# facebookresearch/rela

Hardware: AMD Instinct MI355X
Metric: env-steps/s (Ape-X Atari 84x84x4, actor tick + learner grad-step) (higher is better)
Workload: dtype f32 (f32 operands as 3 exact bf16 parts on bf16 MFMA; f32-accurate); 1 GPU; Ape-X DQN 80x80 envs/GPU, actor+learner on one MI355X, replay 2^20, B=512, A=18, n=3; device-resident static frames; parallelism=single

## Files before the change

### rela_amd/csrc/learner.hip

```cpp
#include "learner_common.h"

using namespace rela_amd;

struct rela_apex_learner {
  int device = 0;
  int A = 0, Bmax = 0;
  float gamma_n = 0.f;
  int optimizer = 0;
  float lr = 0.f, opt_eps = 0.f, clip = 0.f;
  int64_t adam_t = 0;
  int64_t off[13] = {0};
  float *P = nullptr, *PT = nullptr, *G = nullptr, *S1 = nullptr, *S2 = nullptr;
  rela_ffnet *online = nullptr, *target = nullptr;
  float *w2p = nullptr, *w3p = nullptr, *wfcp = nullptr;
  void *ws_on = nullptr, *ws_tmp = nullptr;
  int64_t ws_bytes = 0;
  float *q = nullptr;
  float *td = nullptr, *d_ha = nullptr, *d_h = nullptr, *d_a3 = nullptr, *d_a2 = nullptr, *d_a1 = nullptr;
  float *col = nullptr;
  float *part = nullptr;
  float *cpart = nullptr;
  float *s32 = nullptr;
  double* npart = nullptr;
  float* norm = nullptr;
  float* loss = nullptr;
  bool loaded = false;
  int pend_B = 0, last_B = 0;
  int pend_rows = 0;
  const uint8_t* pend_obs = nullptr;
  hipStream_t side = nullptr;
  hipEvent_t ev[8] = {nullptr};
  float *part_side = nullptr, *cpart_side = nullptr;
  void *frag2 = nullptr, *frag3 = nullptr;
};

namespace {
rela_ffnet_params params_at(const rela_apex_learner* l, float* base) {
  rela_ffnet_params p;
  const float** f = reinterpret_cast<const float**>(&p);
  for (int i = 0; i < 12; ++i) f[i] = base + l->off[i];
  return p;
}

int repack(rela_apex_learner* l, bool online, bool target, hipStream_t s) {
  if (online) {
    const rela_ffnet_params p = params_at(l, l->P);
    FFNetExtraPacks extra;
    extra.w2p = l->w2p, extra.w3p = l->w3p, extra.wfcp = l->wfcp;
    int rc = ffnet_load_extra(l->online, &p, s, extra);
    if (rc != RELA_OK) return rc;
    if (l->frag2) dgfast::pack_frags(l->w2p, l->w3p, l->frag2, l->frag3, s);
  }
  if (target) {
    const rela_ffnet_params p = params_at(l, l->PT);
    int rc = rela_ffnet_load(l->target, &p, 1, s);
    if (rc != RELA_OK) return rc;
  }
  return RELA_OK;
}
}

extern "C" int rela_apex_learner_create(rela_apex_learner** out, int num_action, int max_batch, int multi_step,
                                        float gamma, int optimizer, float lr, float eps, float grad_clip,
                                        int device) {
  RELA_CHECK(out && num_action >= 1 && num_action <= 31 && max_batch >= 1 && multi_step >= 1 &&
                 (optimizer == 0 || optimizer == 1),
             RELA_EINVAL, "rela_apex_learner_create: bad arguments (A=%d batch=%d n=%d optimizer=%d)", num_action,
             max_batch, multi_step, optimizer);
  int ndev = 0;
  if (hipGetDeviceCount(&ndev) != hipSuccess || device < 0 || device >= ndev) {
    set_last_error("rela_apex_learner_create: HIP device %d not available (%d visible); there is no CPU path",
                   device, ndev);
    return RELA_ENODEV;
  }
  DeviceGuard g(device);
  auto* l = new rela_apex_learner();
  l->device = device;
  l->A = num_action;
  l->Bmax = max_batch;
  l->gamma_n = (float)pow((double)gamma, (double)multi_step);
  l->optimizer = optimizer;
  l->lr = lr;
  l->opt_eps = eps;
  l->clip = grad_clip;
  const int64_t cnt[12] = {32 * 256, 32, 64 * 512, 64, 64 * 576, 64, (int64_t)512 * 3136, 512, 512, 1,
                           (int64_t)num_action * 512, num_action};
  for (int i = 0; i < 12; ++i) l->off[i + 1] = l->off[i] + (cnt[i] + 3) / 4 * 4;
  const size_t nb = sizeof(float) * (size_t)l->off[12];
  const size_t B = (size_t)max_batch, A = (size_t)num_action;
  RELA_HIP(hipMalloc(&l->P, nb));
  RELA_HIP(hipMalloc(&l->PT, nb));
  RELA_HIP(hipMalloc(&l->G, nb));
  RELA_HIP(hipMalloc(&l->S1, nb));
  RELA_HIP(hipMalloc(&l->S2, nb));
  RELA_HIP(hipMemset(l->P, 0, nb));
  RELA_HIP(hipMemset(l->PT, 0, nb));
  RELA_HIP(hipMemset(l->G, 0, nb));
  RELA_HIP(hipMemset(l->S1, 0, nb));
  RELA_HIP(hipMemset(l->S2, 0, nb));
  int rc = rela_ffnet_create(&l->online, num_action, device);
  if (rc != RELA_OK) return rc;
  rc = rela_ffnet_create(&l->target, num_action, device);
  if (rc != RELA_OK) return rc;
  ffnet_label_as_learner(l->online);
  ffnet_label_as_learner(l->target);
  ffnet_set_max_rows(l->online, max_batch);
  ffnet_set_max_rows(l->target, max_batch);
  RELA_HIP(hipMalloc(&l->w2p, sizeof(float) * 64 * 512));
  RELA_HIP(hipMalloc(&l->w3p, sizeof(float) * 64 * 576));
  RELA_HIP(hipMalloc(&l->wfcp, sizeof(float) * 512 * 3136));
  l->ws_bytes = std::max(rela_ffnet_workspace_bytes(nullptr, max_batch), rela_ffnet_workspace_bytes(nullptr, 2 * max_batch));
  RELA_HIP(hipMalloc(&l->ws_on, (size_t)l->ws_bytes));
  RELA_HIP(hipMalloc(&l->ws_tmp, (size_t)l->ws_bytes));
  RELA_HIP(hipMalloc(&l->q, sizeof(float) * 3 * B * A));
  RELA_HIP(hipMalloc(&l->td, sizeof(float) * B));
  RELA_HIP(hipMalloc(&l->d_ha, sizeof(float) * B * 32));
  RELA_HIP(hipMalloc(&l->d_h, sizeof(float) * B * 512));
  RELA_HIP(hipMalloc(&l->d_a3, sizeof(float) * B * kA3));
  RELA_HIP(hipMalloc(&l->d_a2, sizeof(float) * B * kA2));
  RELA_HIP(hipMalloc(&l->d_a1, sizeof(float) * B * kA1));
  RELA_HIP(hipMalloc(&l->col, sizeof(float) * trunk_col_floats(B)));
  RELA_HIP(hipMalloc(&l->part, sizeof(float) * kTrunkPartFloats));
  RELA_HIP(hipMalloc(&l->cpart, sizeof(float) * kColsumBlocks * (32 + 512 + 64 + 64 + 32)));
  RELA_HIP(hipMalloc(&l->s32, sizeof(float) * 32));
  RELA_HIP(hipMalloc(&l->npart, sizeof(double) * kNormBlocks));
  RELA_HIP(hipMalloc(&l->norm, sizeof(float) * 2));
  RELA_HIP(hipMalloc(&l->loss, sizeof(float)));
  static const bool lanes = !(getenv("RELA_LEARNER_LANES") && atoi(getenv("RELA_LEARNER_LANES")) == 1);
  if (lanes) {
    RELA_HIP(hipStreamCreateWithFlags(&l->side, hipStreamNonBlocking));
    for (hipEvent_t& e : l->ev) RELA_HIP(hipEventCreateWithFlags(&e, hipEventDisableTiming));
    RELA_HIP(hipMalloc(&l->part_side, sizeof(float) * kTrunkPartFloats));
    RELA_HIP(hipMalloc(&l->cpart_side, sizeof(float) * kColsumBlocks * (32 + 512 + 64 + 64 + 32)));
    RELA_HIP(hipMalloc(&l->frag2, dgfast::kFrag2Bytes));
    RELA_HIP(hipMalloc(&l->frag3, dgfast::kFrag3Bytes));
  }
  *out = l;
  return RELA_OK;
}

extern "C" void rela_apex_learner_destroy(rela_apex_learner* l) {
  if (!l) return;
  DeviceGuard g(l->device);
  (void)hipDeviceSynchronize();
  void* ps[] = {l->P,  l->PT,   l->G,    l->S1,   l->S2,   l->w2p, l->w3p,  l->wfcp,  l->ws_on, l->ws_tmp, l->q,
                l->td, l->d_ha, l->d_h,  l->d_a3, l->d_a2, l->d_a1, l->col, l->part,  l->cpart, l->s32,    l->npart,
                l->norm, l->loss, l->part_side, l->cpart_side, l->frag2, l->frag3};
  for (void* p : ps) (void)hipFree(p);
  for (hipEvent_t e : l->ev)
    if (e) (void)hipEventDestroy(e);
  if (l->side) (void)hipStreamDestroy(l->side);
  rela_ffnet_destroy(l->online);
  rela_ffnet_destroy(l->target);
  delete l;
// ... 196 lines not shown
    ProbHeadWgrad p{};
    p.M = 32, p.N = 512, p.K = Bn;
    p.d_ha = l->d_ha, p.h = w.h, p.g_a_w = Gm[10], p.g_v_w = Gm[8], p.A = A;
    if (g3) (void)gemm3::launch_gemm<Tile3W32>(p, 1, sw, "learner_wgrad_heads");
    else if (g6) (void)gemm3::launch_gemm<Tile6W32>(p, 1, sw, "learner_wgrad_heads");
    else launch_gemm<TileW32>(p, 1, sw, "learner_wgrad_heads");
  }
  sums.add(l->d_ha, Bn, 32, l->s32);
  if (lanes) lane_dep(l->ev[3], s, sw);
  {
    ProbFcDgrad p{};
    p.M = Bn, p.N = 3136, p.K = 512;
    p.d_h = l->d_h, p.wfcp = l->wfcp, p.a3 = w.a3, p.d_a3 = l->d_a3;
    if (g3) (void)gemm3::launch_gemm<Tile3Dgrad>(p, 1, s, "learner_dgrad_fc");
    else if (g6) (void)gemm3::launch_gemm<Tile6Dgrad>(p, 1, s, "learner_dgrad_fc");
    else launch_gemm<TileDgrad>(p, 1, s, "learner_dgrad_fc");
  }
  {
    ProbFcWgrad p{};
    p.M = 512, p.N = 3136, p.K = Bn;
    p.d_h = l->d_h, p.a3 = w.a3, p.g_fc_w = Gm[6];
    if (g3) (void)gemm3::launch_gemm<Tile3Wfc>(p, 1, sw, "learner_wgrad_fc");
    else if (g6) (void)gemm3::launch_gemm<Tile6Wfc>(p, 1, sw, "learner_wgrad_fc");
    else launch_gemm<TileWfc>(p, 1, sw, "learner_wgrad_fc");
  }
  sums.add(l->d_h, Bn, 512, Gm[7]);
  {
    TrunkBwd t{};
    t.Bn = Bn, t.obs = obs, t.a1 = w.a1, t.a2 = w.a2, t.d_a3 = l->d_a3, t.d_a2 = l->d_a2, t.d_a1 = l->d_a1;
    t.col = l->col, t.part = l->part, t.cpart = l->cpart, t.w2p = l->w2p, t.w3p = l->w3p;
    t.g_c1w = Gm[0], t.g_c1b = Gm[1], t.g_c2w = Gm[2], t.g_c2b = Gm[3], t.g_c3w = Gm[4], t.g_c3b = Gm[5];
    t.fast = rela_ffnet_precision(l->online) == 1;
    t.emu = g6;
    if (lanes) {
      t.side = sw, t.ev_da3 = l->ev[4], t.ev_da2 = l->ev[5], t.ev_side = l->ev[6];
      t.part_side = l->part_side, t.cpart_side = l->cpart_side;
      if (t.fast) t.frag2 = l->frag2, t.frag3 = l->frag3;
      t.s32 = l->s32, t.A = A, t.g_a_b = Gm[11], t.g_v_b = Gm[9];
    }
    trunk_backward(t, s, &sums);
    if (!lanes) hipLaunchKernelGGL(head_bias_grad, dim3(1), dim3(32), 0, s, (const float*)l->s32, A, Gm[11], Gm[9]);
  }
  RELA_LAUNCH_CHECK();
  return RELA_OK;
}

extern "C" int rela_apex_learner_apply(rela_apex_learner* l, void* stream_) {
  RELA_CHECK(l && l->loaded, RELA_ESTATE, "rela_apex_learner_apply: parameters were never loaded");
  hipStream_t s = (hipStream_t)stream_;
  DeviceGuard g(l->device);
  OptimState o;
  o.optimizer = l->optimizer, o.lr = l->lr, o.eps = l->opt_eps, o.clip = l->clip, o.adam_t = l->adam_t;
  optimizer_apply(o, l->P, l->G, l->S1, l->S2, l->off[12], l->npart, l->norm, s);
  l->adam_t = o.adam_t;
  RELA_LAUNCH_CHECK();
  return repack(l, true, false, s);
}
```

### rela_amd/csrc/learner_common.h

```cpp
#pragma once
#include <cmath>
#include <cstring>
#include <vector>

#include "common.h"
#include "ffnet_layout.h"
#include "gemm_lds.h"
#include "gemm_bf16x3.h"
#include "prof.h"
#include "dgrad_conv_bf16.h"
#include "wgrad_conv1_bf16.h"
#include "wgrad_conv2_bf16.h"
#include "wgrad_conv3_bf16.h"

namespace rela_amd {
namespace {

using namespace gemm;

using TileDgrad = TileCfg<128, 64, 4, 2, false>;
using TileWfc = TileCfg<128, 64, 4, 2, true>;
using TileW64 = TileCfg<64, 64, 2, 4, true>;
using TileW32 = TileCfg<32, 64, 2, 4, true>;
using Tile3Dgrad = gemm3::TileCfg<128, 64, 4, 2, false>;
using Tile3Wfc = gemm3::TileCfg<128, 64, 4, 2, true>;
using Tile3W64 = gemm3::TileCfg<64, 64, 2, 4, true>;
using Tile3W32 = gemm3::TileCfg<32, 64, 2, 4, true>;
inline bool gemm_bf16x3_on() { return true; }
using Tile6Dgrad = gemm3::TileCfg<128, 64, 4, 2, false, 3>;
using Tile6Wfc = gemm3::TileCfg<128, 64, 4, 2, true, 3>;
using Tile6W64 = gemm3::TileCfg<64, 64, 2, 4, true, 3>;
using Tile6W32 = gemm3::TileCfg<32, 64, 2, 4, true, 3>;


struct ProbHeadDgrad : ProbBase {
  const float *d_ha, *a_w, *v_w, *h;
  float* d_h;
  int A;
  __device__ float4 loadA(int m, int k) const { return m < M ? ld4(d_ha + (size_t)m * 32 + k) : zero4(); }
  __device__ float4 loadB(int k, int n) const {
    if (k < A) return ld4(a_w + (size_t)k * 512 + n);
    if (k == 31) return ld4(v_w + n);
    return zero4();
// ... 426 lines not shown
  reinterpret_cast<float4*>(sq)[i] = sv;
  reinterpret_cast<float4*>(p)[i] = pv;
}
__global__ void adam_update(float* __restrict__ p, const float* __restrict__ g, float* __restrict__ m1,
                            float* __restrict__ m2, int64_t n4, float lr, float b1, float b2, float eps, float bc1,
                            float bc2_sqrt, const float* __restrict__ coef) {
  const int64_t i = (int64_t)blockIdx.x * blockDim.x + threadIdx.x;
  const float cf = coef[1];
  if (i >= n4 || cf < 0.f) return;
  const float4 gv = reinterpret_cast<const float4*>(g)[i];
  float4 av = reinterpret_cast<float4*>(m1)[i], bv = reinterpret_cast<float4*>(m2)[i], pv = reinterpret_cast<float4*>(p)[i];
  auto upd = [&](float gi, float& a, float& b, float& pi) {
    gi = gi * cf;
    a = b1 * a + (1.0f - b1) * gi;
    b = b2 * b + (1.0f - b2) * gi * gi;
    pi -= (lr / bc1) * (a / (sqrtf(b) / bc2_sqrt + eps));
  };
  upd(gv.x, av.x, bv.x, pv.x), upd(gv.y, av.y, bv.y, pv.y), upd(gv.z, av.z, bv.z, pv.z), upd(gv.w, av.w, bv.w, pv.w);
  reinterpret_cast<float4*>(m1)[i] = av;
  reinterpret_cast<float4*>(m2)[i] = bv;
  reinterpret_cast<float4*>(p)[i] = pv;
}


constexpr int kSplitW3 = 28, kSplitW2 = 27, kSplitW1 = 64;
constexpr size_t kTrunkPartFloats = (size_t)w3fast::kMaxBlocks * 64 * 576;
static_assert(kTrunkPartFloats * 4 >= dgfast::kFrag3Bytes && kTrunkPartFloats * 4 >= dgfast::kFrag2Bytes, "frag scratch");
static_assert(kTrunkPartFloats >= (size_t)kSplitW3 * 8 * 64 * 576, "part size (split multiplier up to 8)");
static_assert(kTrunkPartFloats >= (size_t)kSplitW3 * 64 * 576 && kTrunkPartFloats >= (size_t)w1fast::kMaxBlocks * 32 * 256 &&
                  kTrunkPartFloats >= (size_t)w2fast::kMaxBlocks * 64 * 512,
              "part size");
static_assert(kSplitW3 * 64 * 576 >= kSplitW2 * 64 * 512 && kSplitW3 * 64 * 576 >= kSplitW1 * 32 * 256, "part size");
inline size_t trunk_col_floats(size_t frames) { return frames * (size_t)(81 * 512 > 49 * 576 ? 81 * 512 : 49 * 576); }

constexpr int kFastWgradMinFrames = 2048;
struct TrunkBwd {
  int Bn;
  const uint8_t* obs;
  const float *a1, *a2;
  const float* d_a3;
  float *d_a2, *d_a1;
  float* col;
  float* part;
  float* cpart;
  const float *w2p, *w3p;
  float *g_c1w, *g_c1b, *g_c2w, *g_c2b, *g_c3w, *g_c3b;
  bool fast = false;
  bool emu = false;
  hipStream_t side = nullptr;
  hipEvent_t ev_da3 = nullptr, ev_da2 = nullptr, ev_side = nullptr;
  float *part_side = nullptr, *cpart_side = nullptr;
  const void *frag2 = nullptr, *frag3 = nullptr;
  const float* s32 = nullptr;
  float *g_a_b = nullptr, *g_v_b = nullptr;
  int A = 0;
};
inline void lane_dep(hipEvent_t ev, hipStream_t from, hipStream_t to) {
  (void)hipEventRecord(ev, from);
  (void)hipStreamWaitEvent(to, ev, 0);
}

inline void colsum_multi_launch(ColsumJobs& jobs, float* cpart, hipStream_t s) {
  if (jobs.n == 0) return;
  int maxC = 0;
  size_t off = 0;
  for (int j = 0; j < jobs.n; ++j) {
    jobs.part[j] = cpart + off;
    off += (size_t)kColsumBlocks * jobs.C[j];
    maxC = jobs.C[j] > maxC ? jobs.C[j] : maxC;
  }
  ProfScope prof("learner_colsum", s);
  hipLaunchKernelGGL(colsum_partial_multi, dim3(kColsumBlocks, jobs.n), dim3(kLT), 0, s, jobs);
  hipLaunchKernelGGL(colsum_final_multi, dim3(maxC / 4, jobs.n), dim3(kColsumBlocks), 0, s, jobs);
}

inline void colsum_launch(const float* src, int64_t rows, int C, float* cpart, float* out, hipStream_t s) {
  ProfScope prof("learner_colsum", s);
  hipLaunchKernelGGL(colsum_partial, dim3(kColsumBlocks), dim3(kLT), 0, s, src, rows, C, cpart);
  hipLaunchKernelGGL(colsum_final, dim3(C / 4), dim3(kColsumBlocks), 0, s, (const float*)cpart, C, out);
}

inline void trunk_backward(const TrunkBwd& t, hipStream_t s, ColsumJobs* pending = nullptr) {
  const int Bn = t.Bn;
  ColsumJobs own;
  ColsumJobs& jobs = pending ? *pending : own;
  const bool lanes = t.side != nullptr;
  hipStream_t sw = lanes ? t.side : s;
  float* partw = lanes ? t.part_side : t.part;
  if (lanes) lane_dep(t.ev_da3, s, sw);
  const bool fast23 = t.fast && Bn >= kFastWgradMinFrames;
  if (fast23) {
    int blocks = 0;
    {
      ProfScope prof("learner_wgrad_conv3", sw);
      (void)w3fast::launch(t.a2, t.d_a3, Bn, partw, sw, &blocks);
    }
    hipLaunchKernelGGL(reduce_splits, dim3(ceil_div(64 * 576, 256)), dim3(256), 0, sw, (const float*)partw, blocks, 64,
                       576, kRedConv3, t.g_c3w);
  } else {
    ProbW3 p{};
    p.M = 64, p.N = 576, p.K = Bn * 49;
    p.d_out = t.d_a3, p.in = t.a2, p.part = partw;
    static const int mul = 3  ;
    const int split3 = Bn <= 1024 ? kSplitW3 * mul : kSplitW3;
    if (t.fast && gemm_bf16x3_on()) (void)gemm3::launch_gemm<Tile3W64>(p, split3, sw, "learner_wgrad_conv3");
    else if (t.emu) (void)gemm3::launch_gemm<Tile6W64>(p, split3, sw, "learner_wgrad_conv3");
    else launch_gemm<TileW64>(p, split3, sw, "learner_wgrad_conv3");
    hipLaunchKernelGGL(reduce_splits, dim3(ceil_div(64 * 576, 256)), dim3(256), 0, sw, (const float*)partw, split3, 64,
                       576, kRedConv3, t.g_c3w);
  }
  jobs.add(t.d_a3, (int64_t)Bn * 49, 64, t.g_c3b);
  if (t.fast) {
    ProfScope prof("learner_dgrad_conv3", s);
    (void)dgfast::launch_conv3(t.d_a3, t.w3p, t.a2, t.d_a2, Bn, t.part, s, t.frag3);
  } else {
    ProbConvDgrad p{};
    p.M = Bn * 49, p.N = 576, p.K = 64;
    p.d_out = t.d_a3, p.wp = t.w3p, p.col = t.col;
    launch_gemm<TileDgrad>(p, 1, s, "learner_dgrad_conv3");
    ProfScope prof("learner_col2im", s);
    hipLaunchKernelGGL(col2im3, dim3(ceil_div((int64_t)Bn * 81 * 16, 256)), dim3(256), 0, s, (const float*)t.col, t.a2,
                       t.d_a2, Bn);
  }
  if (lanes) lane_dep(t.ev_da2, s, sw);
  if (fast23) {
    int blocks = 0;
    {
      ProfScope prof("learner_wgrad_conv2", sw);
      (void)w2fast::launch(t.a1, t.d_a2, Bn, partw, sw, &blocks);
    }
    hipLaunchKernelGGL(reduce_splits, dim3(ceil_div(64 * 512, 256)), dim3(256), 0, sw, (const float*)partw, blocks, 64,
                       512, kRedConv2, t.g_c2w);
  } else {
    ProbW2 p{};
    p.M = 64, p.N = 512, p.K = Bn * 81;
    p.d_out = t.d_a2, p.in = t.a1, p.part = partw;
    static const int mul = 3  ;
    const int split2 = Bn <= 1024 ? kSplitW2 * mul : kSplitW2;
    if (t.fast && gemm_bf16x3_on()) (void)gemm3::launch_gemm<Tile3W64>(p, split2, sw, "learner_wgrad_conv2");
    else if (t.emu) (void)gemm3::launch_gemm<Tile6W64>(p, split2, sw, "learner_wgrad_conv2");
    else launch_gemm<TileW64>(p, split2, sw, "learner_wgrad_conv2");
    hipLaunchKernelGGL(reduce_splits, dim3(ceil_div(64 * 512, 256)), dim3(256), 0, sw, (const float*)partw, split2, 64,
                       512, kRedConv2, t.g_c2w);
  }
  jobs.add(t.d_a2, (int64_t)Bn * 81, 64, t.g_c2b);
  if (lanes) {
    colsum_multi_launch(jobs, t.cpart_side, sw);
    if (t.s32) hipLaunchKernelGGL(head_bias_grad, dim3(1), dim3(32), 0, sw, t.s32, t.A, t.g_a_b, t.g_v_b);
    jobs.n = 0;
  }
  if (t.fast) {
    ProfScope prof("learner_dgrad_conv2", s);
    (void)dgfast::launch_conv2(t.d_a2, t.w2p, t.a1, t.d_a1, Bn, t.part, s, t.frag2);
  } else {
    ProbConvDgrad p{};
    p.M = Bn * 81, p.N = 512, p.K = 64;
    p.d_out = t.d_a2, p.wp = t.w2p, p.col = t.col;
    launch_gemm<TileDgrad>(p, 1, s, "learner_dgrad_conv2");
    ProfScope prof("learner_col2im", s);
    hipLaunchKernelGGL(col2im2, dim3(ceil_div((int64_t)Bn * 400 * 8, 256)), dim3(256), 0, s, (const float*)t.col, t.a1,
                       t.d_a1, Bn);
  }
  if (t.fast) {
    int blocks = 0;
    {
      ProfScope prof("learner_wgrad_conv1", s);
      (void)w1fast::launch(t.obs, t.d_a1, Bn, t.part, s, &blocks, lanes ? 128 : w1fast::kMaxBlocks);
    }
    hipLaunchKernelGGL(reduce_splits, dim3(ceil_div(32 * 256, 256)), dim3(256), 0, s, (const float*)t.part, blocks, 32,
                       256, kRedConv1, t.g_c1w);
  } else {
    ProbW1 p{};
    p.M = 32, p.N = 256, p.K = Bn * 400;
    p.d_out = t.d_a1, p.obs = t.obs, p.part = t.part;
    if (t.emu) (void)gemm3::launch_gemm<Tile6W32>(p, kSplitW1, s, "learner_wgrad_conv1");
    else launch_gemm<TileW32>(p, kSplitW1, s, "learner_wgrad_conv1");
    hipLaunchKernelGGL(reduce_splits, dim3(ceil_div(32 * 256, 256)), dim3(256), 0, s, (const float*)t.part, kSplitW1, 32,
                       256, kRedConv1, t.g_c1w);
  }
  jobs.add(t.d_a1, (int64_t)Bn * 400, 32, t.g_c1b);
  colsum_multi_launch(jobs, t.cpart, s);
  if (lanes) lane_dep(t.ev_side, sw, s);
}

struct OptimState {
  int optimizer = 0;
  float lr = 0.f, eps = 0.f, clip = 0.f;
  int64_t adam_t = 0;
};
inline void optimizer_apply(OptimState& o, float* P, const float* G, float* S1, float* S2, int64_t n, double* npart,
                            float* norm, hipStream_t s, const unsigned* abort_word = nullptr) {
  ProfScope prof("learner_optimizer", s);
// ... 18 lines not shown
```

### rela_amd/csrc/learner_r2d2.hip

```cpp
#include "gemm_bf16s.h"
#include "learner_common.h"

using namespace rela_amd;

namespace rela_amd {
namespace {

constexpr int kHid = 512, kGates = 2048, kFeat = 3136;
constexpr int kRecSplitF = 4;
constexpr int kRecSplitB = 8;

using TileRows = TileCfg<128, 64, 4, 2, false>;
using TileRec = TileCfg<64, 64, 2, 4, false>;
using TileWg = TileCfg<128, 64, 4, 2, true>;
using TileW32r = TileCfg<32, 64, 2, 4, true>;

struct ProbGateX : ProbBase {
  const float *a3, *wihT, *bias;
  float* gx;
  __device__ float4 loadA(int m, int k) const { return m < M ? ld4(a3 + (size_t)m * kFeat + k) : zero4(); }
  __device__ float4 loadB(int k, int n) const { return ld4(wihT + (size_t)k * kGates + n); }
  __device__ void store(int, int m, int n, float v) const { gx[(size_t)m * kGates + n] = v + bias[n]; }
};
struct ProbRecFwd : ProbBase {
// ... 473 lines not shown
  const int idx = blockIdx.x * blockDim.x + threadIdx.x;
  if (idx >= rows * 32) return;
  const int r = idx >> 5, k = idx & 31;
  const float g = dqa[r];
  float v = 0.f;
  if (k < A) v = legal[(size_t)r * A + k] * (g * ((k == (int)act[r] ? 1.0f : 0.0f) - 1.0f / (float)A));
  if (k == 31) v = g;
  d_ha[idx] = v;
}

}
}

struct rela_r2d2_learner {
  int device = 0;
  int A = 0, Bmax = 0, seq = 0, burn = 0, n = 0, T = 0;
  float gamma_n = 0.f, eta = 0.f, one_minus_eta = 0.f;
  OptimState opt;
  int64_t off[15] = {0};
  float *P = nullptr, *PT = nullptr, *G = nullptr, *S1 = nullptr, *S2 = nullptr;
  rela_lstmnet *online = nullptr, *target = nullptr;
  float *w2p = nullptr, *w3p = nullptr;
  float *wihT[2] = {nullptr, nullptr}, *whhT[2] = {nullptr, nullptr}, *bsum[2] = {nullptr, nullptr};
  float* wihp = nullptr;
  float *a1 = nullptr, *a2 = nullptr, *a3 = nullptr;
  float* gxs[2] = {nullptr, nullptr};
  float*& gx = gxs[0];
  float *Hs[2] = {nullptr, nullptr}, *Cs[2] = {nullptr, nullptr};
  float* rec_part = nullptr;
  unsigned* rec_bar = nullptr;
  unsigned* rec_chain_bar = nullptr;
  bool rec_chains_fit = true;
  bool rec_persist = true;
  int precision = 0;
  uint8_t* wrec[2] = {nullptr, nullptr};
  uint8_t* wTrec = nullptr;
  uint8_t *arec = nullptr, *trec = nullptr;
  uint64_t wver[2] = {1, 1}, rec_ver[2] = {0, 0};
  uint8_t* s3rec = nullptr;
  void* wx3[2] = {nullptr, nullptr};
  uint64_t x3_ver[2] = {0, 0};
  float *ha = nullptr, *q_on = nullptr, *q_tg = nullptr;
  float *qmin = nullptr, *qa_on = nullptr, *qa_tg = nullptr, *dqa = nullptr, *d_ha = nullptr, *d_o = nullptr;
  float *dc_rec = nullptr;
  float *d_a3 = nullptr, *d_a2 = nullptr, *d_a1 = nullptr, *col = nullptr, *part = nullptr, *cpart = nullptr,
        *s32 = nullptr;
  double* npart = nullptr;
  float *norm = nullptr, *loss = nullptr, *loss_seq = nullptr;
  bool loaded = false;
  int pend_B = 0;
  const uint8_t* pend_obs = nullptr;
};

namespace {
const int64_t* seg_counts(int A, int64_t cnt[14]) {
  const int64_t c[14] = {32 * 256, 32, 64 * 512, 64, 64 * 576, 64, (int64_t)kGates * kFeat, (int64_t)kGates * kHid,
                         kGates, kGates, 512, 1, (int64_t)A * 512, A};
  for (int i = 0; i < 14; ++i) cnt[i] = c[i];
  return cnt;
}

rela_lstmnet_params lparams_at(const rela_r2d2_learner* l, float* base) {
  rela_lstmnet_params p;
  const float** f = reinterpret_cast<const float**>(&p);
  for (int i = 0; i < 14; ++i) f[i] = base + l->off[i];
  return p;
// ... 148 lines not shown
    }
    ca.term = term, ca.tmo = l->rec_bar, ca.bar = l->rec_chain_bar, ca.T = T, ca.Tpad = Tpad, ca.Bn = Bn, ca.burn = burn;
    ProfScope prof("learner_lstm_rec_persist", s);
    hipLaunchKernelGGL(lstm_rec_chain<true>, dim3(8 * kChainBlocks), dim3(kRecThreads), 0, s, ca);
    RELA_LAUNCH_CHECK();
  } else {
    rc = forward_rec_steps(l, 1, Bn, term, false, s);
    if (rc != RELA_OK) return rc;
    rc = forward_rec_steps(l, 0, Bn, term, true, s);
    if (rc != RELA_OK) return rc;
  }
  const size_t blk = (size_t)Bn * kHid;
  rc = lstmnet_heads(l->target, Tt * Bn, l->Hs[1] + (size_t)(burn + 1) * blk, legal_train, l->ha, l->q_tg, s,
                     "learner_fwd_heads");
  if (rc != RELA_OK) return rc;
  return lstmnet_heads(l->online, Tt * Bn, l->Hs[0] + (size_t)(burn + 1) * blk, legal_train, l->ha, l->q_on, s,
                       "learner_fwd_heads");
}
}

extern "C" int rela_r2d2_learner_create(rela_r2d2_learner** out, int num_action, int max_batch, int multi_step,
                                        float gamma, int seq_len, int burn_in, double eta, int optimizer, float lr,
                                        float eps, float grad_clip, int device) {
  RELA_CHECK(out && num_action >= 1 && num_action <= 31 && max_batch >= 1 && max_batch <= 1024 && multi_step >= 1 &&
                 seq_len >= 1 && burn_in >= 0 && (optimizer == 0 || optimizer == 1),
             RELA_EINVAL, "rela_r2d2_learner_create: bad arguments (A=%d batch=%d n=%d seq=%d burn=%d optimizer=%d)",
             num_action, max_batch, multi_step, seq_len, burn_in, optimizer);
  int ndev = 0;
  if (hipGetDeviceCount(&ndev) != hipSuccess || device < 0 || device >= ndev) {
    set_last_error("rela_r2d2_learner_create: HIP device %d not available (%d visible); there is no CPU path", device,
                   ndev);
    return RELA_ENODEV;
  }
  DeviceGuard g(device);
  auto* l = new rela_r2d2_learner();
  l->device = device;
  l->A = num_action, l->Bmax = max_batch, l->seq = seq_len, l->burn = burn_in, l->n = multi_step;
  l->T = burn_in + seq_len + multi_step;
  l->gamma_n = (float)pow((double)gamma, (double)multi_step);
  l->eta = (float)eta;
  l->one_minus_eta = (float)(1.0 - eta);
  l->opt.optimizer = optimizer, l->opt.lr = lr, l->opt.eps = eps, l->opt.clip = grad_clip;
  int64_t cnt[14];
  seg_counts(num_action, cnt);
  for (int i = 0; i < 14; ++i) l->off[i + 1] = l->off[i] + (cnt[i] + 3) / 4 * 4;
  const size_t nb = sizeof(float) * (size_t)l->off[14];
  const size_t B = (size_t)max_batch, A = (size_t)num_action, T = (size_t)l->T, Tt = T - burn_in;
  const size_t rowsAll = T * B, rowsTr = Tt * B;
  auto alloc = [&](float** p, size_t floats, bool zero) -> int {
    RELA_HIP(hipMalloc(p, sizeof(float) * floats));
    if (zero) RELA_HIP(hipMemset(*p, 0, sizeof(float) * floats));
    return RELA_OK;
  };
#define R2_ALLOC(ptr, floats, zero)               \
  do {                                            \
    int _rc = alloc(&(ptr), (floats), (zero));    \
    if (_rc != RELA_OK) return _rc;               \
  } while (0)
  R2_ALLOC(l->P, l->off[14], true);
  R2_ALLOC(l->PT, l->off[14], true);
  R2_ALLOC(l->G, l->off[14], true);
  R2_ALLOC(l->S1, l->off[14], true);
  R2_ALLOC(l->S2, l->off[14], true);
  (void)nb;
  int rc = rela_lstmnet_create(&l->online, num_action, device);
  if (rc != RELA_OK) return rc;
  rc = rela_lstmnet_create(&l->target, num_action, device);
  if (rc != RELA_OK) return rc;
  R2_ALLOC(l->w2p, 64 * 512, false);
// ... 38 lines not shown
    const size_t f = (size_t)kRecSplitF * B * kGates, b = (size_t)kRecSplitB * B * kHid;
    R2_ALLOC(l->rec_part, f > b ? f : b, false);
  }
  RELA_HIP(hipMalloc(&l->rec_bar, sizeof(unsigned) * (size_t)(8 + 2 * ((T + 3) / 4 * 4))));
  RELA_HIP(hipMemset(l->rec_bar, 0, sizeof(unsigned) * (size_t)(8 + 2 * ((T + 3) / 4 * 4))));
  RELA_HIP(hipMalloc(&l->rec_chain_bar, sizeof(unsigned) * (size_t)(8 * ((T + 3) / 4 * 4))));
  l->rec_persist = !(getenv("RELA_R2D2_REC") && strcmp(getenv("RELA_R2D2_REC"), "steps") == 0);
  if (l->rec_persist) {
    int cus = 0;
    RELA_HIP(hipDeviceGetAttribute(&cus, hipDeviceAttributeMultiprocessorCount, device));
    int occ_c = 0, occ_d = 0;
    if (hipOccupancyMaxActiveBlocksPerMultiprocessor(&occ_c, lstm_rec_chain<true>, kRecThreads, 0) != hipSuccess) occ_c = 0;
    if (hipOccupancyMaxActiveBlocksPerMultiprocessor(&occ_d, lstm_bptt_chain<false>, kRecThreads, 0) != hipSuccess) occ_d = 0;
    auto room = [cus](int occ) { return (int64_t)cus * (occ >= 4 ? occ - 1 : occ); };
    if (room(occ_c) < 8 * kChainBlocks || room(occ_d) < 8 * kBpttBlocks) {
      fprintf(stderr, "rela_r2d2_learner_create: %d CUs x (%d, %d) resident blocks cannot hold the persistent recurrent "
                      "grids (%d, %d): using the per-step launches\n", cus, occ_c, occ_d, 8 * kChainBlocks, 8 * kBpttBlocks);
      l->rec_chains_fit = false;
    }
  }
  R2_ALLOC(l->ha, rowsTr * 32, false);
  R2_ALLOC(l->q_on, rowsTr * A, false);
  R2_ALLOC(l->q_tg, rowsTr * A, false);
  R2_ALLOC(l->qmin, 4, false);
  R2_ALLOC(l->qa_on, rowsTr, false);
  R2_ALLOC(l->qa_tg, rowsTr, false);
  R2_ALLOC(l->dqa, rowsTr, false);
  R2_ALLOC(l->d_ha, rowsTr * 32, false);
  R2_ALLOC(l->d_o, rowsTr * kHid, false);
  R2_ALLOC(l->dc_rec, B * kHid, false);
  R2_ALLOC(l->d_a3, rowsTr * kA3, false);
  R2_ALLOC(l->d_a2, rowsTr * kA2, false);
  R2_ALLOC(l->d_a1, rowsTr * kA1, false);
  R2_ALLOC(l->col, trunk_col_floats(rowsTr), false);
  R2_ALLOC(l->part, kTrunkPartFloats, false);
  R2_ALLOC(l->cpart, (size_t)kColsumBlocks * kGates, false);
  R2_ALLOC(l->s32, 32, false);
  R2_ALLOC(l->norm, 2, true);
  R2_ALLOC(l->loss, 1, true);
  R2_ALLOC(l->loss_seq, B, true);
#undef R2_ALLOC
  RELA_HIP(hipMalloc(&l->npart, sizeof(double) * kNormBlocks));
  *out = l;
  return RELA_OK;
}

extern "C" void rela_r2d2_learner_destroy(rela_r2d2_learner* l) {
  if (!l) return;
  DeviceGuard g(l->device);
  (void)hipDeviceSynchronize();
  void* ps[] = {l->P,      l->PT,     l->G,       l->S1,      l->S2,      l->w2p,     l->w3p,   l->wihT[0], l->wihT[1],
                l->whhT[0], l->whhT[1], l->bsum[0], l->bsum[1], l->Hs[0],   l->Hs[1],   l->Cs[0], l->Cs[1],   l->wihp,
                l->a1,    l->a2,      l->a3,      l->gx,      l->rec_part, l->ha,   l->q_on,    l->q_tg,
                l->qmin,   l->qa_on,  l->qa_tg,   l->dqa,     l->d_ha,    l->d_o,     l->dc_rec, l->d_a3,   l->d_a2,
                l->d_a1,   l->col,    l->part,    l->cpart,   l->s32,     l->npart,   l->norm,  l->loss,    l->loss_seq};
  for (void* p : ps) (void)hipFree(p);
  (void)hipFree(l->rec_bar);
  (void)hipFree(l->rec_chain_bar);
  (void)hipFree(l->gxs[1]);
  (void)hipFree(l->wrec[0]);
  (void)hipFree(l->wrec[1]);
  (void)hipFree(l->wTrec);
  (void)hipFree(l->arec);
  (void)hipFree(l->s3rec);
  (void)hipFree(l->wx3[0]);
  (void)hipFree(l->wx3[1]);
  (void)hipFree(l->trec);
// ... 233 lines not shown
    rc = launch_rec64_nt(dgT, a3T, kGates, kHid, chunks, EpiPlain{Gm[7], kHid}, s, "learner_wgrad_lstm_hh");
    if (rc != RELA_OK) return rc;
  } else {
    ProbWih p{};
    p.M = kGates, p.N = kFeat, p.K = rowsTr;
    p.dg = DG, p.a3 = a3_tr, p.out = Gm[6];
    launch_gemm<TileWg>(p, 1, s, "learner_wgrad_lstm_ih");
  }
  colsum_launch(DG, rowsTr, kGates, l->cpart, Gm[8], s);
  RELA_HIP(hipMemcpyAsync(Gm[9], Gm[8], sizeof(float) * kGates, hipMemcpyDeviceToDevice, s));
  if (l->precision == 1) {
    using namespace gemm16;
    {
      ProfScope prof("learner_lstm_split_rows", s);
      hipLaunchKernelGGL(split_rows_rec64, dim3(ceil_div((int64_t)rowsTr * kGates / 8, 256)), dim3(256), 0, s, DG,
                         (int64_t)rowsTr, kGates, l->arec);
    }
    int rc = launch_rec64_nt(l->arec, l->wTrec, rowsTr, kFeat, kGates / 64, EpiReluMask{l->d_a3, a3_tr, kFeat}, s,
                             "learner_dgrad_lstm_ih");
    if (rc != RELA_OK) return rc;
  } else {
    ProbIhDgrad p{};
    p.M = rowsTr, p.N = kFeat, p.K = kGates;
    p.dg = DG, p.wihp = l->wihp, p.a3 = a3_tr, p.d_a3 = l->d_a3;
    launch_gemm<TileRows>(p, 1, s, "learner_dgrad_lstm_ih");
  }
  {
    TrunkBwd t{};
    t.Bn = rowsTr, t.obs = obs + tr0 * 28224, t.a1 = l->a1 + tr0 * kA1, t.a2 = l->a2 + tr0 * kA2, t.d_a3 = l->d_a3;
    t.d_a2 = l->d_a2, t.d_a1 = l->d_a1, t.col = l->col, t.part = l->part, t.cpart = l->cpart;
    t.w2p = l->w2p, t.w3p = l->w3p;
    t.g_c1w = Gm[0], t.g_c1b = Gm[1], t.g_c2w = Gm[2], t.g_c2b = Gm[3], t.g_c3w = Gm[4], t.g_c3b = Gm[5];
    t.fast = l->precision == 1;
    trunk_backward(t, s);
  }
  RELA_LAUNCH_CHECK();
  return RELA_OK;
}

extern "C" int rela_r2d2_learner_apply(rela_r2d2_learner* l, void* stream_) {
  RELA_CHECK(l && l->loaded, RELA_ESTATE, "rela_r2d2_learner_apply: parameters were never loaded");
  hipStream_t s = (hipStream_t)stream_;
  DeviceGuard g(l->device);
  optimizer_apply(l->opt, l->P, l->G, l->S1, l->S2, l->off[14], l->npart, l->norm, s, l->rec_bar);
  RELA_LAUNCH_CHECK();
  return repack_r2d2(l, true, false, s);
}
```

Baseline: 3.315 million env-steps/s.

## Fuse conv2/conv3 dgrad GEMM with col2im in an f32 MFMA kernel

Adds persistent f32 MFMA kernels for the conv3 and conv2 data-gradient that compute each frame's column tile into LDS and then do the col2im scatter-sum and ReLU mask in the same kernel. This becomes the default non-fast path, replacing the tiled GEMM that writes a large global col buffer followed by a separate col2im launch. The aim is to remove that global round-trip and one launch per layer. The old path stays available via RELA_LEARNER_DGRAD=col, and the col buffer is now allocated only in that mode. The trade-off is the native f32 MFMA rate and a per-frame LDS barrier schedule, in place of the tuned GEMM.

After: 3.327 million env-steps/s, median of 2. Within noise of the previous version (+0.4%).

```diff
diff --git a/rela_amd/csrc/dgrad_conv_f32.h b/rela_amd/csrc/dgrad_conv_f32.h
--- /dev/null
+++ b/rela_amd/csrc/dgrad_conv_f32.h
@@ -0,0 +1,200 @@
+#pragma once
+#include <hip/hip_runtime.h>
+
+#include "common.h"
+#include "prof.h"
+
+namespace rela_amd {
+namespace dgf32 {
+namespace {
+
+typedef float f32x4 __attribute__((ext_vector_type(4)));
+
+constexpr int kT = 256;
+constexpr int kFrameLanes = 128;
+
+template <int MT, int M>
+__device__ __forceinline__ void load_a(float (&a)[MT][16], const float* __restrict__ fd, int mt0, int li, int kk) {
+#pragma unroll
+  for (int t = 0; t < MT; ++t) {
+    const int row = min((mt0 + t) * 16 + li, M - 1);
+    const float* p = fd + row * 64 + kk;
+#pragma unroll
+    for (int ks = 0; ks < 16; ++ks) a[t][ks] = p[4 * ks];
+  }
+}
+
+template <int MT, int NT>
+__device__ __forceinline__ void mfma_tiles(const float (&a)[MT][16], const float (&b)[NT][16], f32x4 (&acc)[MT][NT]) {
+#pragma unroll
+  for (int t = 0; t < MT; ++t)
+#pragma unroll
+    for (int u = 0; u < NT; ++u) acc[t][u] = f32x4{0.f, 0.f, 0.f, 0.f};
+#pragma unroll
+  for (int ks = 0; ks < 16; ++ks)
+#pragma unroll
+    for (int t = 0; t < MT; ++t)
+#pragma unroll
+      for (int u = 0; u < NT; ++u) acc[t][u] = __builtin_amdgcn_mfma_f32_16x16x4f32(a[t][ks], b[u][ks], acc[t][u], 0, 0, 0);
+}
+
+struct D3 {
+  static constexpr int M = 49, LDC = 9 * 16 + 4;
+  static constexpr int ITEMS = 81 * 4, IT = (ITEMS + kT - 1) / kT;
+};
+__global__ __launch_bounds__(kT, 2) void dgrad_conv3_f32(const float* __restrict__ d_a3, const float* __restrict__ w3p,
+                                                         const float* __restrict__ a2, float* __restrict__ d_a2,
+                                                         int frames) {
+  __shared__ __attribute__((aligned(16))) float col[D3::M * D3::LDC];
+  const int tid = threadIdx.x;
+  const int wave = tid >> 6, lane = tid & 63;
+  const int li = lane & 15, kk = lane >> 4;
+  const int cs = blockIdx.x & 3, stride = gridDim.x >> 2;
+  float b[9][16];
+#pragma unroll
+  for (int u = 0; u < 9; ++u)
+#pragma unroll
+    for (int ks = 0; ks < 16; ++ks) b[u][ks] = w3p[(4 * ks + kk) * 576 + u * 64 + 16 * cs + li];
+  int f = blockIdx.x >> 2;
+  float a[1][16];
+  load_a<1, D3::M>(a, d_a3 + (size_t)f * (49 * 64), wave, li, kk);
+  for (; f < frames; f += stride) {
+    f32x4 am[D3::IT];
+#pragma unroll
+    for (int j = 0; j < D3::IT; ++j) {
+      const int i = min(tid + j * kT, D3::ITEMS - 1);
+      am[j] = *reinterpret_cast<const f32x4*>(a2 + ((size_t)f * 81 + (i >> 2)) * 64 + 16 * cs + 4 * (i & 3));
+    }
+    f32x4 acc[1][9];
+    mfma_tiles<1, 9>(a, b, acc);
+    {
+      const int fn = f + stride < frames ? f + stride : f;
+      load_a<1, D3::M>(a, d_a3 + (size_t)fn * (49 * 64), wave, li, kk);
+    }
+#pragma unroll
+    for (int r = 0; r < 4; ++r) {
+      const int row = wave * 16 + 4 * kk + r;
+      if (row < D3::M) {
+#pragma unroll
+        for (int u = 0; u < 9; ++u) col[row * D3::LDC + u * 16 + li] = acc[0][u][r];
+      }
+    }
+    __syncthreads();
+#pragma unroll
+    for (int j = 0; j < D3::IT; ++j) {
+      const int i = tid + j * kT;
+      if (i < D3::ITEMS) {
+        const int c4 = i & 3, pix = i >> 2;
+        const int y = pix / 9, x = pix - y * 9;
+        f32x4 s = {0.f, 0.f, 0.f, 0.f};
+        for (int kh = 0; kh < 3; ++kh) {
+          const int oy = y - kh;
+          if (oy < 0 || oy >= 7) continue;
+          for (int kw = 0; kw < 3; ++kw) {
+            const int ox = x - kw;
+            if (ox < 0 || ox >= 7) continue;
+            const f32x4 v = *reinterpret_cast<const f32x4*>(&col[(oy * 7 + ox) * D3::LDC + (kh * 3 + kw) * 16 + c4 * 4]);
+            s.x += v.x, s.y += v.y, s.z += v.z, s.w += v.w;
+          }
+        }
+        const f32x4 m = am[j];
+        f32x4 d;
+#pragma unroll
+        for (int rr = 0; rr < 4; ++rr) d[rr] = m[rr] > 0.f ? s[rr] : 0.f;
+        *reinterpret_cast<f32x4*>(d_a2 + ((size_t)f * 81 + pix) * 64 + 16 * cs + 4 * c4) = d;
+      }
+    }
+    __syncthreads();
+  }
+}
+
+struct D2 {
+  static constexpr int M = 81, LDC = 4 * 32 + 4;
+  static constexpr int ITEMS = 100 * 8, IT = (ITEMS + kT - 1) / kT;
+};
+__global__ __launch_bounds__(kT, 2) void dgrad_conv2_f32(const float* __restrict__ d_a2, const float* __restrict__ w2p,
+                                                         const float* __restrict__ a1, float* __restrict__ d_a1,
+                                                         int frames) {
+  __shared__ __attribute__((aligned(16))) float col[D2::M * D2::LDC];
+  const int tid = threadIdx.x;
+  const int wave = tid >> 6, lane = tid & 63;
+  const int li = lane & 15, kk = lane >> 4;
+  const int cls = blockIdx.x & 3, stride = gridDim.x >> 2;
+  const int s = cls >> 1, r = cls & 1;
+  const int h = wave & 1, mt0 = 3 * (wave >> 1);
+  float b[4][16];
+#pragma unroll
+  for (int u = 0; u < 4; ++u)
+#pragma unroll
+    for (int ks = 0; ks < 16; ++ks)
+      b[u][ks] = w2p[(4 * ks + kk) * 512 + ((2 * (u >> 1) + s) * 4 + 2 * (u & 1) + r) * 32 + 16 * h + li];
+  int f = blockIdx.x >> 2;
+  float a[3][16];
+  load_a<3, D2::M>(a, d_a2 + (size_t)f * (81 * 64), mt0, li, kk);
+  for (; f < frames; f += stride) {
+    f32x4 am[D2::IT];
+#pragma unroll
+    for (int j = 0; j < D2::IT; ++j) {
+      const int i = min(tid + j * kT, D2::ITEMS - 1);
+      const int pix = i >> 3, u = pix / 10, v = pix - u * 10;
+      am[j] = *reinterpret_cast<const f32x4*>(a1 + ((size_t)f * 400 + (2 * u + s) * 20 + 2 * v + r) * 32 + 4 * (i & 7));
+    }
+    f32x4 acc[3][4];
+    mfma_tiles<3, 4>(a, b, acc);
+    {
+      const int fn = f + stride < frames ? f + stride : f;
+      load_a<3, D2::M>(a, d_a2 + (size_t)fn * (81 * 64), mt0, li, kk);
+    }
+#pragma unroll
+    for (int t = 0; t < 3; ++t)
+#pragma unroll
+      for (int rr = 0; rr < 4; ++rr) {
+        const int row = (mt0 + t) * 16 + 4 * kk + rr;
+        if (row < D2::M) {
+#pragma unroll
+          for (int u = 0; u < 4; ++u) col[row * D2::LDC + u * 32 + 16 * h + li] = acc[t][u][rr];
+        }
+      }
+    __syncthreads();
+#pragma unroll
+    for (int j = 0; j < D2::IT; ++j) {
+      const int i = tid + j * kT;
+      if (i < D2::ITEMS) {
+        const int c4 = i & 7, pix = i >> 3;
+        const int u = pix / 10, v = pix - u * 10;
+        f32x4 sum = {0.f, 0.f, 0.f, 0.f};
+        for (int p = 0; p < 2; ++p) {
+          const int oy = u - p;
+          if (oy < 0 || oy > 8) continue;
+          for (int q = 0; q < 2; ++q) {
+            const int ox = v - q;
+            if (ox < 0 || ox > 8) continue;
+            const f32x4 w = *reinterpret_cast<const f32x4*>(&col[(oy * 9 + ox) * D2::LDC + (2 * p + q) * 32 + c4 * 4]);
+            sum.x += w.x, sum.y += w.y, sum.z += w.z, sum.w += w.w;
+          }
+        }
+        const f32x4 m = am[j];
+        f32x4 d;
+#pragma unroll
+        for (int rr = 0; rr < 4; ++rr) d[rr] = m[rr] > 0.f ? sum[rr] : 0.f;
+        *reinterpret_cast<f32x4*>(d_a1 + ((size_t)f * 400 + (2 * u + s) * 20 + 2 * v + r) * 32 + 4 * c4) = d;
+      }
+    }
+    __syncthreads();
+  }
+}
+
+inline void launch_conv3(const float* d_a3, const float* w3p, const float* a2, float* d_a2, int frames, hipStream_t s) {
+  note_launch("dgrad_conv3_f32");
+  hipLaunchKernelGGL(dgrad_conv3_f32, dim3(4 * (frames < kFrameLanes ? frames : kFrameLanes)), dim3(kT), 0, s, d_a3, w3p,
+                     a2, d_a2, frames);
+}
+inline void launch_conv2(const float* d_a2, const float* w2p, const float* a1, float* d_a1, int frames, hipStream_t s) {
+  note_launch("dgrad_conv2_f32");
+  hipLaunchKernelGGL(dgrad_conv2_f32, dim3(4 * (frames < kFrameLanes ? frames : kFrameLanes)), dim3(kT), 0, s, d_a2, w2p,
+                     a1, d_a1, frames);
+}
+
+}
+}
+}
diff --git a/rela_amd/csrc/learner.hip b/rela_amd/csrc/learner.hip
--- a/rela_amd/csrc/learner.hip
+++ b/rela_amd/csrc/learner.hip
@@ -17,6 +17,7 @@
   int64_t ws_bytes = 0;
   float *q = nullptr;
   float *td = nullptr, *d_ha = nullptr, *d_h = nullptr, *d_a3 = nullptr, *d_a2 = nullptr, *d_a1 = nullptr;
+  bool dgrad_col = false;
   float *col = nullptr;
   float *part = nullptr;
   float *cpart = nullptr;
@@ -73,8 +74,11 @@
                    device, ndev);
     return RELA_ENODEV;
   }
+  const int dgrad = dgrad_col_from_env();
+  RELA_CHECK(dgrad >= 0, RELA_EINVAL, "rela_apex_learner_create: RELA_LEARNER_DGRAD must be \"fused\" or \"col\"");
   DeviceGuard g(device);
   auto* l = new rela_apex_learner();
+  l->dgrad_col = dgrad == 1;
   l->device = device;
   l->A = num_action;
   l->Bmax = max_batch;
@@ -119,7 +123,7 @@
   RELA_HIP(hipMalloc(&l->d_a3, sizeof(float) * B * kA3));
   RELA_HIP(hipMalloc(&l->d_a2, sizeof(float) * B * kA2));
   RELA_HIP(hipMalloc(&l->d_a1, sizeof(float) * B * kA1));
-  RELA_HIP(hipMalloc(&l->col, sizeof(float) * trunk_col_floats(B)));
+  if (l->dgrad_col) RELA_HIP(hipMalloc(&l->col, sizeof(float) * trunk_col_floats(B)));
   RELA_HIP(hipMalloc(&l->part, sizeof(float) * kTrunkPartFloats));
   RELA_HIP(hipMalloc(&l->cpart, sizeof(float) * kColsumBlocks * (32 + 512 + 64 + 64 + 32)));
   RELA_HIP(hipMalloc(&l->s32, sizeof(float) * 32));
@@ -382,6 +386,7 @@
     t.g_c1w = Gm[0], t.g_c1b = Gm[1], t.g_c2w = Gm[2], t.g_c2b = Gm[3], t.g_c3w = Gm[4], t.g_c3b = Gm[5];
     t.fast = rela_ffnet_precision(l->online) == 1;
     t.emu = g6;
+    t.dgrad_col = l->dgrad_col;
     if (lanes) {
       t.side = sw, t.ev_da3 = l->ev[4], t.ev_da2 = l->ev[5], t.ev_side = l->ev[6];
       t.part_side = l->part_side, t.cpart_side = l->cpart_side;
diff --git a/rela_amd/csrc/learner_common.h b/rela_amd/csrc/learner_common.h
--- a/rela_amd/csrc/learner_common.h
+++ b/rela_amd/csrc/learner_common.h
@@ -9,6 +9,7 @@
 #include "gemm_bf16x3.h"
 #include "prof.h"
 #include "dgrad_conv_bf16.h"
+#include "dgrad_conv_f32.h"
 #include "wgrad_conv1_bf16.h"
 #include "wgrad_conv2_bf16.h"
 #include "wgrad_conv3_bf16.h"
@@ -501,6 +502,11 @@
               "part size");
 static_assert(kSplitW3 * 64 * 576 >= kSplitW2 * 64 * 512 && kSplitW3 * 64 * 576 >= kSplitW1 * 32 * 256, "part size");
 inline size_t trunk_col_floats(size_t frames) { return frames * (size_t)(81 * 512 > 49 * 576 ? 81 * 512 : 49 * 576); }
+inline int dgrad_col_from_env() {
+  const char* e = getenv("RELA_LEARNER_DGRAD");
+  if (!e || !*e || strcmp(e, "fused") == 0) return 0;
+  return strcmp(e, "col") == 0 ? 1 : -1;
+}
 
 constexpr int kFastWgradMinFrames = 2048;
 struct TrunkBwd {
@@ -516,6 +522,7 @@
   float *g_c1w, *g_c1b, *g_c2w, *g_c2b, *g_c3w, *g_c3b;
   bool fast = false;
   bool emu = false;
+  bool dgrad_col = false;
   hipStream_t side = nullptr;
   hipEvent_t ev_da3 = nullptr, ev_da2 = nullptr, ev_side = nullptr;
   float *part_side = nullptr, *cpart_side = nullptr;
@@ -582,12 +589,16 @@
   if (t.fast) {
     ProfScope prof("learner_dgrad_conv3", s);
     (void)dgfast::launch_conv3(t.d_a3, t.w3p, t.a2, t.d_a2, Bn, t.part, s, t.frag3);
+  } else if (!t.dgrad_col) {
+    ProfScope prof("learner_dgrad_conv3", s);
+    dgf32::launch_conv3(t.d_a3, t.w3p, t.a2, t.d_a2, Bn, s);
   } else {
     ProbConvDgrad p{};
     p.M = Bn * 49, p.N = 576, p.K = 64;
     p.d_out = t.d_a3, p.wp = t.w3p, p.col = t.col;
     launch_gemm<TileDgrad>(p, 1, s, "learner_dgrad_conv3");
     ProfScope prof("learner_col2im", s);
+    note_launch("col2im3");
     hipLaunchKernelGGL(col2im3, dim3(ceil_div((int64_t)Bn * 81 * 16, 256)), dim3(256), 0, s, (const float*)t.col, t.a2,
                        t.d_a2, Bn);
   }
@@ -621,12 +632,16 @@
   if (t.fast) {
     ProfScope prof("learner_dgrad_conv2", s);
     (void)dgfast::launch_conv2(t.d_a2, t.w2p, t.a1, t.d_a1, Bn, t.part, s, t.frag2);
+  } else if (!t.dgrad_col) {
+    ProfScope prof("learner_dgrad_conv2", s);
+    dgf32::launch_conv2(t.d_a2, t.w2p, t.a1, t.d_a1, Bn, s);
   } else {
     ProbConvDgrad p{};
     p.M = Bn * 81, p.N = 512, p.K = 64;
     p.d_out = t.d_a2, p.wp = t.w2p, p.col = t.col;
     launch_gemm<TileDgrad>(p, 1, s, "learner_dgrad_conv2");
     ProfScope prof("learner_col2im", s);
+    note_launch("col2im2");
     hipLaunchKernelGGL(col2im2, dim3(ceil_div((int64_t)Bn * 400 * 8, 256)), dim3(256), 0, s, (const float*)t.col, t.a1,
                        t.d_a1, Bn);
   }
diff --git a/rela_amd/csrc/learner_r2d2.hip b/rela_amd/csrc/learner_r2d2.hip
--- a/rela_amd/csrc/learner_r2d2.hip
+++ b/rela_amd/csrc/learner_r2d2.hip
@@ -529,6 +529,7 @@
   unsigned* rec_chain_bar = nullptr;
   bool rec_chains_fit = true;
   bool rec_persist = true;
+  bool dgrad_col = false;
   int precision = 0;
   uint8_t* wrec[2] = {nullptr, nullptr};
   uint8_t* wTrec = nullptr;
@@ -743,9 +744,12 @@
                    ndev);
     return RELA_ENODEV;
   }
+  const int dgrad = dgrad_col_from_env();
+  RELA_CHECK(dgrad >= 0, RELA_EINVAL, "rela_r2d2_learner_create: RELA_LEARNER_DGRAD must be \"fused\" or \"col\"");
   DeviceGuard g(device);
   auto* l = new rela_r2d2_learner();
   l->device = device;
+  l->dgrad_col = dgrad == 1;
   l->A = num_action, l->Bmax = max_batch, l->seq = seq_len, l->burn = burn_in, l->n = multi_step;
   l->T = burn_in + seq_len + multi_step;
   l->gamma_n = (float)pow((double)gamma, (double)multi_step);
@@ -850,7 +854,7 @@
   R2_ALLOC(l->d_a3, rowsTr * kA3, false);
   R2_ALLOC(l->d_a2, rowsTr * kA2, false);
   R2_ALLOC(l->d_a1, rowsTr * kA1, false);
-  R2_ALLOC(l->col, trunk_col_floats(rowsTr), false);
+  if (l->dgrad_col) R2_ALLOC(l->col, trunk_col_floats(rowsTr), false);
   R2_ALLOC(l->part, kTrunkPartFloats, false);
   R2_ALLOC(l->cpart, (size_t)kColsumBlocks * kGates, false);
   R2_ALLOC(l->s32, 32, false);
@@ -1150,6 +1154,7 @@
     t.w2p = l->w2p, t.w3p = l->w3p;
     t.g_c1w = Gm[0], t.g_c1b = Gm[1], t.g_c2w = Gm[2], t.g_c2b = Gm[3], t.g_c3w = Gm[4], t.g_c3b = Gm[5];
     t.fast = l->precision == 1;
+    t.dgrad_col = l->dgrad_col;
     trunk_backward(t, s);
   }
   RELA_LAUNCH_CHECK();
```
